# sea-with-sakura/ViT-of-Pytorch

Measured on AMD Instinct MI355X. Metric: images/sec training step, ViT-B/16 224px bf16, 1/2/4/8 MI355X, higher is better.
Workload: dtype bf16; 1 GPU; ViT-B16 @224 train step (fwd+CE+bwd+SGD-momentum/OneCycleLR); model=ViT-B16, image_size=224, per_gpu_batch=256, global_batch=256, seq_len=197, num_classes=1000, parallelism=dp1, step_launch=eager

## Files before the change

include/vit_hip.h:

```cpp
#ifndef VIT_HIP_H_
#define VIT_HIP_H_

#include <stdint.h>

#ifdef __cplusplus
extern "C" {
#endif

typedef void* vit_stream_t;

enum vit_status {
  VIT_OK = 0,
  VIT_ERR_INVALID_ARG = 1,
  VIT_ERR_HIP = 2,
  VIT_ERR_UNSUPPORTED = 3,
};

const char* vit_last_error(void);
int vit_abi_version(void);
const char* vit_build_id(void);

enum vit_layout { VIT_K_CONTIG = 0, VIT_MN_CONTIG = 1 };

typedef struct vit_dropout {
// ... 43 lines not shown
  int64_t batch;
  int64_t split_k;
  int64_t tokens;
  float* col_partial;
  int32_t epilogue;
  int32_t tile;
  const vit_dropout* dropout;
} vit_gemm_args;

int vit_gemm_bf16(const vit_gemm_args* args, vit_stream_t stream);
int64_t vit_gemm_tile_rows(const vit_gemm_args* args);
int64_t vit_gemm_partial_rows(const vit_gemm_args* args);
int64_t vit_gemm_split_rows(const vit_gemm_args* args);
int vit_gemm_bf16_part(const vit_gemm_args* args, int32_t part, vit_stream_t stream);
int vit_gemm_splitk_group(const vit_gemm_args* args, int32_t n, vit_stream_t stream);

int vit_splitk_reduce(const float* ws, int64_t batch, int64_t split, int64_t M, int64_t N,
                      float* out, int64_t ldo, int64_t out_batch_stride, int32_t accumulate,
                      vit_stream_t stream);
#define VIT_SPLITK_GROUP_MAX 8
typedef struct vit_splitk_job {
  const float* ws;
  int64_t batch, split, M, N;
  float* out;
  int64_t ldo, out_batch_stride;
  int32_t accumulate;
  int32_t reserved;
} vit_splitk_job;
int vit_splitk_reduce_group(const vit_splitk_job* jobs, int32_t njobs, vit_stream_t stream);

// ... 162 lines not shown
```

vit-of-pytorch_amd/csrc/capi.hip:

```cpp
#include <stdarg.h>

#include "common.h"
#include "build_id.h"

namespace vit {
static thread_local char g_last_error[512] = "";

void set_error(const char* fmt, ...) {
  va_list ap;
  va_start(ap, fmt);
  vsnprintf(g_last_error, sizeof(g_last_error), fmt, ap);
  va_end(ap);
}

int check_hip(hipError_t e, const char* what) {
  if (e == hipSuccess) return VIT_OK;
  set_error("%s: %s", what, hipGetErrorString(e));
  return VIT_ERR_HIP;
}
}

extern "C" const char* vit_last_error(void) { return vit::g_last_error; }
extern "C" int vit_abi_version(void) { return 20; }
extern "C" const char* vit_build_id(void) { return VIT_BUILD_ID; }
```

vit-of-pytorch_amd/csrc/gemm.hip:

```cpp
#include "gemm_decl.h"

namespace {
using vitg::GemmDev;
using vitg::EPI_DROP;

int pick_tile(const vit_gemm_args* a) {
  if (a->tile > 0) return (int)a->tile;
  const bool ak = a->a_layout == VIT_K_CONTIG, bk = a->b_layout == VIT_K_CONTIG;
  if (a->epilogue == VIT_EPI_SPLITK && a->M >= 256 && a->N >= 256) {
    static const int env_sk = vit::knob("VIT_GEMM_SPLITK_CFG", 9);
    return env_sk == 5 || env_sk == 6 || env_sk == 7 || env_sk == 8 ? env_sk : 9;
  }
  if (a->M >= 1024 && a->N >= 256) {
    static const int env_rs = vit::knob("VIT_GEMM_RESID_PP2", 1);
    if (ak && (env_rs || !(a->epilogue == VIT_EPI_BIAS_RESID_F32 && a->K < 2048))) return 9;
    if (a->N >= 2048 && a->epilogue != VIT_EPI_GELU_BWD && a->epilogue != VIT_EPI_MUL_BF16) return 5;
    if (!bk && a->K >= 3072) return 5;
    return 3;
  }
  return 0;
}

int tile_rows_of(int cfg) {
  switch (cfg) {
// ... 99 lines not shown
  d.B = (const char*)a->B; d.ldb = a->ldb; d.b_bs = a->b_batch_stride; d.b_bytes = (uint32_t)b_bytes;
  d.C = a->C; d.ldc = a->ldc; d.c_bs = a->c_batch_stride;
  d.C2 = a->C2; d.ldc2 = a->ldc2;
  d.bias = a->bias; d.bias_bs = a->bias_batch_stride;
  d.aux = a->aux; d.ldaux = a->ldaux; d.aux2 = a->aux2;
  d.split_k = (int)a->split_k; d.tokens = (int)a->tokens;
  {
    auto al = [](const void* q) { return ((uintptr_t)q % 32) == 0; };
    bool v = al(a->C) && a->ldc % 8 == 0 && a->c_batch_stride % 8 == 0;
    if (a->C2) v = v && al(a->C2) && a->ldc2 % 8 == 0;
    if (a->bias) v = v && al(a->bias) && a->bias_batch_stride % 8 == 0;
    if (a->aux) v = v && al(a->aux) && a->ldaux % 8 == 0;
    if (a->aux2) v = v && al(a->aux2);
    if (a->epilogue == VIT_EPI_SPLITK) v = al(a->C) && a->N % 8 == 0;
    d.vec = v ? 1 : 0;
  }
  d.col_partial = a->col_partial;
  d.drop = make_drop(a->dropout);
  VIT_CHECK_ARG(!d.drop.thr || a->epilogue == VIT_EPI_PATCH || a->epilogue == VIT_EPI_BIAS_RESID_F32 ||
                    a->epilogue == VIT_EPI_BIAS_GELU_DGELU,
                "vit_gemm_bf16: dropout is supported on the PATCH, BIAS_RESID_F32 and BIAS_GELU_DGELU epilogues");
  VIT_CHECK_ARG(!d.drop.thr || (a->a_layout == VIT_K_CONTIG &&
                                  (a->b_layout == VIT_K_CONTIG || a->epilogue == VIT_EPI_BIAS_RESID_F32)),
                "vit_gemm_bf16: dropout epilogues need a K-contiguous A (and B, except BIAS_RESID_F32)");
  {
    static const int env_gm = vit::knob("VIT_GEMM_GROUP_M", 8);
    static const int env_nt = vit::knob("VIT_GEMM_NT", 0);
    d.group_m = env_gm;
    d.nt = env_nt;
    static const int env_diag = vit::knob("VIT_GEMM_DIAG", 0);
// ... 98 lines not shown
    const vit_gemm_args* a = args + i;
    VIT_CHECK_ARG(a->epilogue == VIT_EPI_SPLITK && a->a_layout == VIT_MN_CONTIG && a->b_layout == VIT_MN_CONTIG &&
                      a->tile == 0 && !a->col_partial && !a->dropout,
                  "vit_gemm_splitk_group: member %d must be a split-K weight gradient (VIT_EPI_SPLITK, both operands "
                  "M/N-contiguous, no tile / col_partial / dropout)", i);
    bool empty = false;
    if (const int rc = make_dev(a, g.g[i], empty)) return rc;
    VIT_CHECK_ARG(!empty, "vit_gemm_splitk_group: member %d is empty", i);
    g.start[i] = (int)total;
    total += ((a->M + 255) / 256) * ((a->N + 255) / 256) * a->split_k * a->batch;
    VIT_CHECK_ARG(total < (1L << 30), "vit_gemm_splitk_group: grid too large");
  }
  g.start[n] = (int)total;
  g.n = n;
  return vit::check_hip(vitg::launch_splitk_group(g, (hipStream_t)stream), "vit_gemm_splitk_group launch");
}

namespace {
__global__ void splitk_reduce_kernel(const float* __restrict__ ws, int split, long M, long N, float* __restrict__ out,
                                     long ldo, long obs, int accumulate) {
  const int z = blockIdx.y;
  const long total = M * N;
  const float* w = ws + (long)z * split * total;
  float* o = out + z * obs;
  for (long i = (long)blockIdx.x * blockDim.x + threadIdx.x; i < total; i += (long)gridDim.x * blockDim.x) {
    float s = 0.f;
    for (int k = 0; k < split; ++k) s += w[k * total + i];
    const long m = i / N, n = i - m * N;
    float* dst = o + m * ldo + n;
    *dst = accumulate ? *dst + s : s;
// ... 135 lines not shown
```

vit-of-pytorch_amd/csrc/gemm_decl.h:

```cpp
#pragma once
#include "common.h"
#include <stdlib.h>

namespace vitg {

struct GemmDev {
  int M, N, K;
  const char* A;
  long lda;
  long a_bs;
  uint32_t a_bytes;
  const char* B;
  long ldb;
  long b_bs;
  uint32_t b_bytes;
  void* C;
  long ldc;
  long c_bs;
  void* C2;
  long ldc2;
  const float* bias;
  long bias_bs;
  const void* aux;
  long ldaux;
// ... 10 lines not shown
  int prio;
  int ilv;
#ifdef VIT_PP2_STAMPS
  unsigned long long* stamps;
#endif
};

constexpr int GEMM_GROUP_MAX = 4;
struct GemmGroup {
  GemmDev g[GEMM_GROUP_MAX];
  int start[GEMM_GROUP_MAX + 1];
  int n;
};
hipError_t launch_splitk_group(const GemmGroup& g, hipStream_t s);

constexpr int EPI_DROP = 16;

template <int EPI>
hipError_t launch_layout_x(int cfg, const GemmDev& d, bool ak, bool bk, int batch, int split, hipStream_t s);
template <int EPI>
hipError_t launch_kk_x(int cfg, const GemmDev& d, bool bk, int batch, int split, hipStream_t s);
template <> hipError_t launch_layout_x<0>(int, const GemmDev&, bool, bool, int, int, hipStream_t);
template <> hipError_t launch_layout_x<1>(int, const GemmDev&, bool, bool, int, int, hipStream_t);
template <> hipError_t launch_layout_x<2>(int, const GemmDev&, bool, bool, int, int, hipStream_t);
template <> hipError_t launch_layout_x<3>(int, const GemmDev&, bool, bool, int, int, hipStream_t);
template <> hipError_t launch_layout_x<4>(int, const GemmDev&, bool, bool, int, int, hipStream_t);
template <> hipError_t launch_layout_x<5>(int, const GemmDev&, bool, bool, int, int, hipStream_t);
template <> hipError_t launch_layout_x<6>(int, const GemmDev&, bool, bool, int, int, hipStream_t);
template <> hipError_t launch_layout_x<7>(int, const GemmDev&, bool, bool, int, int, hipStream_t);
template <> hipError_t launch_layout_x<8>(int, const GemmDev&, bool, bool, int, int, hipStream_t);
// ... 7 lines not shown
```

vit-of-pytorch_amd/csrc/gemm_e7.hip:

```cpp
#include "gemm_kernels.h"

template <> hipError_t vitg::launch_layout_x<7>(int cfg, const GemmDev& d, bool ak, bool bk, int batch, int split, hipStream_t s) {
  return launch_layout<7>(cfg, d, ak, bk, batch, split, s);
}

hipError_t vitg::launch_splitk_group(const GemmGroup& g, hipStream_t s) { return launch_pp2_group(g, s); }
```

vit-of-pytorch_amd/csrc/gemm_kernels.h:

```cpp
#pragma once
#include "gemm_decl.h"

namespace {
using vitg::GemmDev;
using vitg::GemmGroup;
using vitg::GEMM_GROUP_MAX;

__device__ __forceinline__ void tile_coords(int wg, int tiles_m, int tiles_n, int gm, int& tm, int& tn) {
  if (gm <= 1) {
    tm = wg / tiles_n;
    tn = wg % tiles_n;
    return;
  }
  const int per = gm * tiles_n;
  const int first = (wg / per) * gm;
  const int rows = tiles_m - first < gm ? tiles_m - first : gm;
  const int r = wg % per;
  tm = first + r % rows;
  tn = r / rows;
}

template <int BK>
__device__ __forceinline__ int swz_k(int row) {
  if constexpr (BK == 64) return (row >> 1) & 7;
// ... 148 lines not shown
    bf16_t* C = (bf16_t*)p.C + z * p.c_bs;
    const bf16_t* U = (const bf16_t*)p.aux;
    C[(long)m * p.ldc + n] = f2bf(v * bf2f(U[(long)m * p.ldaux + n]));
  } else if constexpr (E == VIT_EPI_PATCH) {
    float* C = (float*)p.C;
    const float* pos = (const float*)p.aux;
    const int t = m % p.tokens;
    float o;
    if (t == 0)
      o = p.aux2[n] + pos[n];
    else
      o = v + p.bias[n] + pos[(long)t * p.ldaux + n];
    if constexpr (DROP) o *= drop_mult1(p.drop, m, n);
    C[(long)m * p.ldc + n] = o;
  } else if constexpr (E == VIT_EPI_SPLITK) {
    float* C = (float*)p.C + ((long)z * p.split_k + split_idx) * (long)p.M * p.N;
    C[(long)m * p.N + n] = v;
  }
}

__device__ __forceinline__ void ld8f(const float* p, float* v) {
  const float4 a = *reinterpret_cast<const float4*>(p);
  const float4 b = *reinterpret_cast<const float4*>(p + 4);
  v[0] = a.x; v[1] = a.y; v[2] = a.z; v[3] = a.w; v[4] = b.x; v[5] = b.y; v[6] = b.z; v[7] = b.w;
}
typedef float v4f_t __attribute__((ext_vector_type(4)));
typedef unsigned v4u_t __attribute__((ext_vector_type(4)));
__device__ __forceinline__ void st8f(float* p, const float* v, bool nt = false) {
  const v4f_t a = {v[0], v[1], v[2], v[3]}, b = {v[4], v[5], v[6], v[7]};
  if (nt) {
    __builtin_nontemporal_store(a, reinterpret_cast<v4f_t*>(p));
    __builtin_nontemporal_store(b, reinterpret_cast<v4f_t*>(p + 4));
// ... 133 lines not shown
#pragma unroll
      for (int k = 0; k < 8; ++k) v[k] = b[k] + ps[k];
    } else {
      ld8f(p.bias + n, b);
#pragma unroll
      for (int k = 0; k < 8; ++k) v[k] += b[k] + ps[k];
    }
    if constexpr (DROP) {
      float dm[8];
      drop_mult8(p.drop, m, n >> 3, dm);
#pragma unroll
      for (int k = 0; k < 8; ++k) v[k] *= dm[k];
    }
    st8f((float*)p.C + (long)m * p.ldc + n, v, p.nt);
  } else if constexpr (E == VIT_EPI_SPLITK) {
    st8f((float*)p.C + ((long)z * p.split_k + split_idx) * (long)p.M * p.N + (long)m * p.N + n, v, p.nt);
  }
}

template <int EPI>
struct EpiOut {
  static constexpr int E = EPI & 15;
  static constexpr int W = (E == VIT_EPI_BF16 || E == VIT_EPI_BIAS_BF16 || E == VIT_EPI_GELU_BWD || E == VIT_EPI_MUL_BF16)
                               ? 1
                               : 2;
  static constexpr bool BIAS = E == VIT_EPI_BIAS_BF16 || E == VIT_EPI_BIAS_GELU || E == VIT_EPI_BIAS_RESID_F32 ||
                               E == VIT_EPI_BIAS_GELU_DGELU;
  static constexpr bool FAST = E != VIT_EPI_PATCH;
};

__device__ __forceinline__ uint4 pack8bf(const float* v) {
// ... 71 lines not shown
  }
}

__device__ __forceinline__ void st16(void* q, const uint4& x, bool nt) {
  const v4u_t u = {x.x, x.y, x.z, x.w};
  if (nt)
    __builtin_nontemporal_store(u, reinterpret_cast<v4u_t*>(q));
  else
    *reinterpret_cast<v4u_t*>(q) = u;
}

template <int EPI>
__device__ __forceinline__ void epi_put8(const GemmDev& p, int z, int split_idx, int m, int n, const uint4* o) {
  constexpr int E = EPI & 15;
  if constexpr (E == VIT_EPI_SPLITK) {
    float* q = (float*)p.C + ((long)z * p.split_k + split_idx) * (long)p.M * p.N + (long)m * p.N + n;
    st16(q, o[0], p.nt);
    st16(q + 4, o[1], p.nt);
  } else if constexpr (EpiOut<EPI>::W == 1) {
    st16((bf16_t*)p.C + z * p.c_bs + (long)m * p.ldc + n, o[0], p.nt);
  } else if constexpr (E == VIT_EPI_BIAS_GELU || E == VIT_EPI_BIAS_GELU_DGELU) {
    st16((bf16_t*)p.C + z * p.c_bs + (long)m * p.ldc + n, o[0], p.nt);
    st16((bf16_t*)p.C2 + z * p.c_bs + (long)m * p.ldc2 + n, o[1], p.nt);
  } else {
    float* q = (float*)p.C + z * p.c_bs + (long)m * p.ldc + n;
    st16(q, o[0], p.nt);
    st16(q + 4, o[1], p.nt);
  }
}

template <int EPI>
// ... 651 lines not shown
```

vit-of-pytorch_amd/csrc/gemm_pp2.inc:

```
template <bool AK, bool BKC, int EPI, int BK = 64, int NA = 2>
__device__ __forceinline__ void pp2_tile(const GemmDev& p, const int tm, const int tn, const int z,
                                         const int split_idx, const int orig) {
  constexpr int BM = 256, BN = 256, KK = BK / 32;
  constexpr int NB = NA + 1;
  constexpr int TN = BN / 4, FM = 8, FN = TN / 16;
  constexpr int HALF = 128 * BK * 2;
  constexpr int A0_OFF = 0, A1_OFF = NA * HALF, B_OFF = 2 * NA * HALF;
  constexpr int LDS = (2 * NA + 2 * NB) * HALF;
  constexpr int I = BK / 16;
  constexpr int LDW = TN + 4;
  constexpr int PR = 32;
  constexpr int WST = PR * LDW * 4;
  static_assert(8 * WST <= LDS && LDS <= 160 * 1024, "LDS budget / epilogue staging");
  static_assert(2 * I * (NA - 1) <= 32 && (2 * NA - 1) * I <= 62 && 2 * (NB - 1) * I <= 62, "vmcnt range");
  __shared__ __attribute__((aligned(16))) char smem[LDS];

  const int lane = threadIdx.x & 63;
  const int wave = __builtin_amdgcn_readfirstlane(threadIdx.x >> 6);
  const int grp = wave >> 2, wn = wave & 3;
  const int m0 = tm * BM, n0 = tn * BN;
  if (p.diag >= 100 && ((orig >> 3) & 1) && (orig >> 3) < 32) {
    const unsigned long long t0 = __builtin_amdgcn_s_memrealtime();
    while (__builtin_amdgcn_s_memrealtime() - t0 < (unsigned long long)(p.diag - 100) * 100ull)
      __builtin_amdgcn_s_sleep(8);
// ... 396 lines not shown
__global__ void __launch_bounds__(512) gemm_pp2_group_kernel(const GemmGroup G) {
  const int orig = blockIdx.x;
  const int w = xcd_major(orig, G.start[G.n]);
  int gi = 0;
#pragma unroll
  for (int k = 1; k < GEMM_GROUP_MAX; ++k)
    if (k < G.n && w >= G.start[k]) gi = k;
  gi = __builtin_amdgcn_readfirstlane(gi);
  const GemmDev& p = G.g[gi];
  const int tiles_m = (p.M + 255) / 256, tiles_n = (p.N + 255) / 256;
  int tm, tn, z, split_idx;
  splitk_coords(p, w - G.start[gi], tiles_m * tiles_n, tiles_m, tiles_n, tm, tn, z, split_idx);
  pp2_tile<AK, BKC, VIT_EPI_SPLITK>(p, tm, tn, z, split_idx, orig);
}

template <bool AK, bool BKC, int EPI, int BK = 64, int NA = 2>
hipError_t launch_pp2(const GemmDev& d, int batch, int split, hipStream_t s) {
  const int tiles = ((d.M + 255) / 256) * ((d.N + 255) / 256);
  dim3 grid(tiles, split, batch);
  hipLaunchKernelGGL((gemm_pp2_kernel<AK, BKC, EPI, BK, NA>), grid, dim3(512), 0, s, d);
  return hipGetLastError();
}

inline hipError_t launch_pp2_group(const GemmGroup& g, hipStream_t s) {
  hipLaunchKernelGGL((gemm_pp2_group_kernel<false, false>), dim3(g.start[g.n]), dim3(512), 0, s, g);
  return hipGetLastError();
}
```

vit-of-pytorch_amd/vitmi/_lib.py:

```python
from __future__ import annotations

import ctypes
import os

_HERE = os.path.dirname(os.path.abspath(__file__))
LIB_PATH = os.environ.get("VITMI_LIB") or os.path.join(_HERE, "libvit_hip.so")

c_i64 = ctypes.c_int64
c_i32 = ctypes.c_int32
c_f32 = ctypes.c_float
c_vp = ctypes.c_void_p

ABI_VERSION = 20

K_CONTIG, MN_CONTIG = 0, 1
(EPI_F32, EPI_BF16, EPI_BIAS_BF16, EPI_BIAS_GELU, EPI_BIAS_RESID_F32, EPI_GELU_BWD, EPI_PATCH, EPI_SPLITK,
 EPI_BIAS_GELU_DGELU, EPI_MUL_BF16) = range(10)


class Dropout(ctypes.Structure):
    _fields_ = [("p", c_f32), ("site", ctypes.c_uint32), ("seed", ctypes.c_uint64), ("offset", ctypes.c_uint64),
                ("row_stride", c_i64)]


class GemmArgs(ctypes.Structure):
    _fields_ = [
        ("M", c_i64), ("N", c_i64), ("K", c_i64),
        ("A", c_vp), ("lda", c_i64), ("a_batch_stride", c_i64),
# ... 28 lines not shown
    _fields_ = [("inp", c_vp), ("rows", c_i64), ("cols", c_i64), ("ldi", c_i64), ("out", c_vp), ("ldo", c_i64),
                ("rows_pad", c_i64), ("cols_pad", c_i64)]


CAST_BATCH_MAX = 8

_SIGS = {
    "vit_last_error": (ctypes.c_char_p, []),
    "vit_abi_version": (c_i32, []),
    "vit_gemm_bf16": (c_i32, [ctypes.POINTER(GemmArgs), c_vp]),
    "vit_gemm_tile_rows": (c_i64, [ctypes.POINTER(GemmArgs)]),
    "vit_gemm_partial_rows": (c_i64, [ctypes.POINTER(GemmArgs)]),
    "vit_gemm_split_rows": (c_i64, [ctypes.POINTER(GemmArgs)]),
    "vit_gemm_bf16_part": (c_i32, [ctypes.POINTER(GemmArgs), c_i32, c_vp]),
    "vit_gemm_splitk_group": (c_i32, [ctypes.POINTER(GemmArgs), c_i32, c_vp]),
    "vit_segment_colsum": (c_i32, [c_vp, c_i32, c_i64, c_i64, c_i64, c_i64, c_i64, c_i64, c_f32, c_vp, c_i64, c_vp]),
    "vit_segment_colsum_bcast": (c_i32, [c_vp, c_i32, c_i64, c_i64, c_i64, c_i64, c_i64, c_i64, c_f32, c_vp, c_i64,
                                         c_vp, c_i64, c_i64, c_vp]),
    "vit_router_dx_gate_partial_rows": (c_i64, [c_i64]),
    "vit_router_dx_gate": (c_i32, [c_vp, c_i64, c_vp, c_i64, c_f32, c_vp, c_i64, c_i64, c_i64, c_i64, c_i64, c_vp,
                                   c_i64, c_i64, c_i64, c_vp, c_i64, c_vp]),
    "vit_splitk_reduce_group": (c_i32, [ctypes.POINTER(SplitkJob), c_i32, c_vp]),
    "vit_cast_pad_batch": (c_i32, [ctypes.POINTER(CastJob), c_i32, c_vp]),
    "vit_router_head_partials": (c_i64, [c_i64]),
    "vit_cast_rows_masked": (c_i32, [c_vp, c_i64, c_i64, c_i64, c_vp, c_vp, c_i64, c_vp]),
    "vit_router_select": (c_i32, [c_vp, c_i64, c_i32, ctypes.POINTER(ctypes.c_uint32), c_i32, c_vp, c_vp, c_vp, c_vp]),
    "vit_cls_mse": (c_i32, [c_vp, c_i64, c_vp, c_i64, c_i64, c_i64, c_vp, c_vp, c_vp, c_vp]),
    "vit_cls_mse_bwd": (c_i32, [c_vp, c_i64, c_vp, c_i64, c_i64, c_vp, c_vp]),
    "vit_router_head_fwd": (c_i32, [c_vp, c_vp, c_i32, c_vp, c_i64, c_i64, c_i32, c_i64, c_i32, c_f32, c_vp, c_vp, c_vp,
                                    c_vp, c_vp, c_vp, c_vp]),
# ... 111 lines not shown
```

vit-of-pytorch_amd/vitmi/engine.py:

```python
from __future__ import annotations

import math
import os
from collections import OrderedDict
from dataclasses import dataclass

import torch

from . import ops
from ._lib import (EPI_BF16, EPI_BIAS_BF16, EPI_BIAS_GELU_DGELU, EPI_BIAS_RESID_F32, EPI_MUL_BF16, EPI_PATCH,
                   EPI_SPLITK, K_CONTIG, MN_CONTIG)

ALIGN = 64


def _rup(x, m):
    return (x + m - 1) // m * m


_NBUF = 2

_WGRAD_TARGET = int(os.environ.get("VIT_WGRAD_TARGET", "256"))


# ... 148 lines not shown
        self.dqkv = [z(Tp, 3 * D), z(Tp, 3 * D)]
        self.dlncls = z(b, D, dt=f)
        self.dlogits = z(b, cfg.num_classes, dt=f)
        self.row_stats = z(b, 3, dt=f)
        self.lnparts = [z(ops.layernorm_bwd_blocks(T), 3 * D, dt=f) for _ in range(_NBUF)]
        self.gelu_parts = [z(-(-T // 128), M, dt=f) for _ in range(_NBUF)]
        self.attn_bias_rows = ops.attention_bias_rows(N, D // H)
        self.qkv_bparts = [z(b * self.attn_bias_rows, 3 * D, dt=f) for _ in range(_NBUF)]
        nws = ops.attention_workspace_elems(b, N, H)
        self.attn_ws = z(nws, dt=f) if nws else None
        bp = _rup(b, 64)
        self.bp = bp
        self.c_o, self.c_ln2, self.c_dh, self.c_dh2, self.c_dyln = (z(bp, D) for _ in range(5))
        self.c_g, self.c_gp, self.c_dg = (z(bp, M) for _ in range(3))
        self.c_mu2, self.c_rs2 = z(b, dt=f), z(b, dt=f)


class _BiasReducer:

    def __init__(self, eng, a):
        self.eng = eng
        self.a = a
        self.D = eng.cfg.emb_dim
        self.nxt = {}
        self.queued = {}
        self.jobs = []

    def buf(self, kind, bufs):
        n = self.queued.get(kind, 0)
        if n == len(bufs):
# ... 47 lines not shown
        self.wqkv = torch.zeros(L, D, 3 * D, device=self.dev, dtype=bf)
        self.bqkv = torch.zeros(L, 3 * D, device=self.dev)
        kp = _rup(cfg.patch_k, 64)
        self.wconv = torch.zeros(D, kp, device=self.dev, dtype=torch.bfloat16) if kp != cfg.patch_k else None
        self._acts = {}
        self._mirror_sig = None
        o = [self.off(self.lname(i, "norm1.weight")) for i in range(L)]
        self.layer_stride = o[0] - o[1] if L > 1 else 0
        assert all(o[i] == o[0] - i * self.layer_stride for i in range(L))
        self._ws = None
        self.step_id = 0
        self.grad_ready_hook = None
        self.grad_ready_finish = None
        self.overlap_wgrad = os.environ.get("VITMI_OVERLAP", "0") == "1"
        self.group_wgrad = os.environ.get("VITMI_GROUP_WGRAD", "1") != "0"
        self.prune_last = os.environ.get("VITMI_PRUNE_LAST", "1") != "0"
        self._pruned = False
        self._side = None
        self._ev_pool, self._ev_next = [], 0
        self.probe = None
        self.probe_wgrad = None
        self.drop_seed = (torch.initial_seed() * 0x9E3779B97F4A7C15 + 0x632BE59BD9B4E019) & (2**64 - 1)
        self._drop_offset = 0
        self._drop = None

    def _event(self):
        if self._ev_next == len(self._ev_pool):
            self._ev_pool.append(torch.cuda.Event())
        ev = self._ev_pool[self._ev_next]
        self._ev_next += 1
# ... 79 lines not shown
            A, lda, B, ldb, M, N, _, _, _, batch, b_bs, _ = sp
            w = ws[o:o + n]
            o += n
            views.append(w)
            members.append((A, B, w, M, N, K, dict(a_layout=MN_CONTIG, b_layout=MN_CONTIG, lda=lda, ldb=ldb, ldc=N,
                                                    epilogue=EPI_SPLITK, batch=batch, b_bs=b_bs, split_k=s)))
        if self.probe_wgrad is not None:
            ev0 = torch.cuda.Event(enable_timing=True)
            ev0.record()
        ops.gemm_splitk_group(members)
        if self.probe_wgrad is not None:
            ev1 = torch.cuda.Event(enable_timing=True)
            ev1.record()
            self.probe_wgrad.append((ev0, ev1, sum(2.0 * sp[4] * sp[5] * K * sp[9] for sp in specs), K, True))
        ops.splitk_reduce_group([(w, sp[9], s, sp[4], sp[5], sp[7], sp[8], sp[11], False) for sp, w in zip(specs, views)])

    def _dd(self, site, row_stride=1):
        if self._drop is None:
            return None
        p, seed, off = self._drop
        return ops.dropout_desc(p, site, seed, off, row_stride)

    def forward(self, x: torch.Tensor, dropout_p: float = 0.0):
        cfg = self.cfg
        if x.dim() != 4 or x.shape[1] != 3 or tuple(x.shape[2:]) != cfg.image_hw:
            raise ValueError(f"expected input [b, 3, {cfg.image_hw[0]}, {cfg.image_hw[1]}], got {tuple(x.shape)}")
        x = x.to(self.dev, torch.float32).contiguous()
        b = x.shape[0]
        a = self.acts(b)
        D, M, H, N, L = cfg.emb_dim, cfg.mlp_dim, cfg.num_heads, cfg.tokens, cfg.num_layers
# ... 185 lines not shown
                main.wait_event(ev)

        def fire(bucket):
            bias.flush()
            if not hook:
                return
            evs = []
            for st in ((main, side) if overlap else (main,)):
                ev = self._event()
                ev.record(st)
                evs.append(ev)
            hook(g, *bucket, evs)

        self._ev_next = 0
        group = self.group_wgrad and D >= 256
        out_wb = None
        bias = _BiasReducer(self, a)
        ops.gemm_f32(C, D, b, dl, C, True, a.lncls, D, False, gv("classifier.weight"), D)
        bias.reduce(dl, b, C, C, (gv("classifier.bias"),))
        ops.gemm_f32(b, D, C, dl, C, False, f[self.off("classifier.weight"):], D, False, a.dlncls, D)
        wb = 0
        pruned = self._pruned
        ops.zero_(a.dh)
        if not pruned:
            ops.zero_(a.dhb[wb])
        bias.ln_bwd(a.dlncls, D, a.h[L], N * D, a.muf, a.rsf, f[self.off("transformer.norm.weight"):], a.dh, N * D, b,
                    gv("transformer.norm.weight"), gv(self.lname(L - 1, "mlp.fc2.bias")),
                    dx_bf16=a.c_dh if pruned else a.dhb[wb], lddxb=D if pruned else N * D,
                    dx_dropout=dd(3 + 3 * (L - 1), N))
        fire(self.layout.buckets[0])
        scale = 1.0 / math.sqrt(hd)
        for i in reversed(range(L)):
            ln = lambda s: self.off(self.lname(i, s))
            li = i & 1
            if pruned and i == L - 1:
                self._backward_last_cls(a, i, b, g, on_side, bias)
                wb ^= 1
            else:
                dhb = a.dhb[wb]
                on_side(lambda: self._wgrad(dhb, D, a.g[i], M, D, M, a.Tp, gv(self.lname(i, "mlp.fc2.weight")), M))
                release("dhb", wb)
                dg = a.dg[li]
                acquire("dg", li)
                gpart = bias.buf("gelu", a.gelu_parts)
                w2 = mv[ln("mlp.fc2.weight"):]
                kw = dict(a_layout=K_CONTIG, b_layout=MN_CONTIG, lda=D, ldb=M, ldc=M, epilogue=EPI_MUL_BF16, aux=a.gp[i],
                          ldaux=M, col_partial=gpart)
                ops.gemm(dhb, w2, dg, T, M, D, **kw)
                tiles_m = ops.gemm_partial_rows(dhb, w2, dg, T, M, D, **kw)
                bias.reduce(gpart, tiles_m, M, M, (gv(self.lname(i, "mlp.fc1.bias")),))
                on_side(lambda: self._wgrad(dg, M, a.ln2[i], D, M, D, a.Tp, gv(self.lname(i, "mlp.fc1.weight")), D))
                release("dg", li)
                ops.gemm(dg, mv[ln("mlp.fc1.weight"):], a.dyln, T, D, M, a_layout=K_CONTIG, b_layout=MN_CONTIG, lda=M,
                         ldb=D, ldc=D, epilogue=EPI_BF16)
                wb ^= 1
                acquire("dhb", wb)
                dhb = a.dhb[wb]
                bias.ln_bwd(a.dyln, D, a.hm[i], D, a.mu2[i], a.rs2[i], f[ln("norm2.weight"):], a.dh, D, T,
                            gv(self.lname(i, "norm2.weight")), gv(self.lname(i, "attn.out.bias")),
                            dres=a.dh, lddres=D, dx_bf16=dhb, lddxb=D, dx_dropout=dd(1 + 3 * i))
                out_spec = (a.o[i], D, dhb, D, D, D, a.Tp, gv(self.lname(i, "attn.out.weight")), D, 1, 0, 0)
                if group:
                    out_wb = wb
                else:
                    on_side(lambda: self._wgrad(*out_spec[:9]))
                    release("dhb", wb)
                ops.gemm(dhb, mv[ln("attn.out.weight"):], a.dO, T, D, D, a_layout=K_CONTIG, b_layout=K_CONTIG, lda=D,
                         ldb=D, ldc=D, epilogue=EPI_BF16)
            dqkv = a.dqkv[li]
            acquire("dqkv", li)
            qpart = bias.buf("qkv", a.qkv_bparts)
            ops.attention_bwd(a.qkv[i], a.o[i], a.dO, a.lse[i], dqkv, b, N, H, hd, scale, bias_partial=qpart,
                              q_rows=1 if pruned and i == L - 1 else None, workspace=a.attn_ws)
            qo = ln("attn.query.weight")
            zs = ln("attn.key.weight") - qo
            qb = ln("attn.query.bias")
            bias.reduce(qpart, b * a.attn_bias_rows, 3 * D, 3 * D, (g[qb:], g[qb + zs:], g[qb + 2 * zs:]), seg=D)
            qkv_spec = (a.ln1[i], D, dqkv, 3 * D, D, D, a.Tp, g[qo:], D, 3, D, zs)
            if out_wb is not None:
                on_side(lambda: self._wgrad_group([out_spec, qkv_spec]))
                release("dqkv", li)
                release("dhb", out_wb)
                out_wb = None
            else:
                on_side(lambda: self._wgrad(*qkv_spec[:9], batch=3, b_bs=D, out_bs=zs))
                release("dqkv", li)
            ops.gemm(dqkv, self.wqkv[i], a.dyln, T, D, 3 * D, a_layout=K_CONTIG, b_layout=K_CONTIG, lda=3 * D,
                     ldb=3 * D, ldc=D, epilogue=EPI_BF16)
            wb ^= 1
            acquire("dhb", wb)
            bias.ln_bwd(a.dyln, D, a.h[i], D, a.mu1[i], a.rs1[i], f[ln("norm1.weight"):], a.dh, D, T,
                        gv(self.lname(i, "norm1.weight")), gv(self.lname(i - 1, "mlp.fc2.bias")) if i > 0 else None,
                        dres=a.dh, lddres=D, dx_bf16=a.dhb[wb], lddxb=D,
                        dx_dropout=dd(3 + 3 * (i - 1)) if i > 0 else dd(0))
            fire(self.layout.buckets[L - i])
        dhb = a.dhb[wb]
        on_side(lambda: self._wgrad(dhb, D, a.patches, a.kpad, D, cfg.patch_k, a.Tp, gv("embedding.weight"),
                                    cfg.patch_k))
        ops.embed_grad(a.dh, b, N, D, gv("transformer.pos_embedding.pos_embedding"), gv("cls_token"),
                       gv("embedding.bias"), dropout=dd(0))
        fire(self.layout.buckets[-1])
        bias.flush()
        if overlap:
            main.wait_stream(side)
        return g
```

vit-of-pytorch_amd/vitmi/ops.py:

```python
from __future__ import annotations

import ctypes

import torch

from . import _lib
from ._lib import COLSUM_BATCH_MAX, Dropout, GemmArgs, check

BF16 = torch.bfloat16
F32 = torch.float32


def lib():
    return _lib.load()


def _stream():
    return ctypes.c_void_p(torch.cuda.current_stream().cuda_stream)


def _p(t):
    return ctypes.c_void_p(0 if t is None else t.data_ptr())


# ... 502 lines not shown
            best, best_t = s, t
    return best


def gemm_splitk_group(members):
    if not 1 <= len(members) <= 4:
        raise ValueError("gemm_splitk_group: 1 to 4 members")
    arr = (GemmArgs * len(members))()
    for i, (A, B, C, M, N, K, kw) in enumerate(members):
        _chk(A, BF16, "A")
        _chk(B, BF16, "B")
        arr[i] = _gemm_args(A, B, C, M, N, K, **kw)
    check(lib().vit_gemm_splitk_group(arr, len(members), _stream()), "vit_gemm_splitk_group")


def splitk_factor(M, N, K, batch=1, cus=256):
    tile = 256 if M >= 256 and N >= 256 else 128
    slots = cus if tile == 256 else 2 * cus
    tiles = -(-M // tile) * -(-N // tile) * batch
    smax = max(1, min((K // 64) // 8, 32))
    t_tile = 2.0 * tile * tile * K / 4.0e12
    slab = 2.0 * M * N * 4 * batch / 5.0e12
    best, best_t = 1, None
    for s in range(1, smax + 1):
        t = -(-tiles * s // slots) * t_tile / s + s * slab
        if best_t is None or t < best_t * (1 - 1e-9):
            best, best_t = s, t
    return best


# ... 28 lines not shown
```

Baseline: 7711 images/sec.

## Defer all weight-gradient GEMMs into one table-driven grouped launch

Weight-gradient GEMMs are no longer launched per layer during backward. They are queued and issued at the end as one grouped kernel. The kernel reads a device-resident table of per-member GEMM descriptors, which is cached across steps and keyed on pointers, and each workgroup finds its member by binary search. Split-K members can now write directly into the gradient buffer through ldc and c_bs. The aim is to cut launch overhead and fill the device with one large grid, at the cost of extra per-layer activation-gradient buffers, serialising wgrad after the dgrad chain, and a host sync whenever the table is rebuilt.

Measured after the change: 7824 images/sec, median of 6. 1.01x the previous value.

```diff
diff --git a/include/vit_hip.h b/include/vit_hip.h
--- a/include/vit_hip.h
+++ b/include/vit_hip.h
@@ -81,6 +81,11 @@
 int64_t vit_gemm_split_rows(const vit_gemm_args* args);
 int vit_gemm_bf16_part(const vit_gemm_args* args, int32_t part, vit_stream_t stream);
 int vit_gemm_splitk_group(const vit_gemm_args* args, int32_t n, vit_stream_t stream);
+#define VIT_GEMM_TABLE_MAX 128
+int64_t vit_gemm_group_table_bytes(int32_t n);
+int vit_gemm_group_prepare(const vit_gemm_args* args, const int32_t* direct, int32_t n, void* table,
+                           int64_t table_bytes, int32_t* total, vit_stream_t stream);
+int vit_gemm_group_launch(const void* table, int32_t n, int32_t total, vit_stream_t stream);
 
 int vit_splitk_reduce(const float* ws, int64_t batch, int64_t split, int64_t M, int64_t N,
                       float* out, int64_t ldo, int64_t out_batch_stride, int32_t accumulate,
diff --git a/vit-of-pytorch_amd/csrc/capi.hip b/vit-of-pytorch_amd/csrc/capi.hip
--- a/vit-of-pytorch_amd/csrc/capi.hip
+++ b/vit-of-pytorch_amd/csrc/capi.hip
@@ -21,5 +21,5 @@
 }
 
 extern "C" const char* vit_last_error(void) { return vit::g_last_error; }
-extern "C" int vit_abi_version(void) { return 20; }
+extern "C" int vit_abi_version(void) { return 21; }
 extern "C" const char* vit_build_id(void) { return VIT_BUILD_ID; }
diff --git a/vit-of-pytorch_amd/csrc/gemm.hip b/vit-of-pytorch_amd/csrc/gemm.hip
--- a/vit-of-pytorch_amd/csrc/gemm.hip
+++ b/vit-of-pytorch_amd/csrc/gemm.hip
@@ -1,4 +1,6 @@
 #include "gemm_decl.h"
+
+#include <vector>
 
 namespace {
 using vitg::GemmDev;
@@ -137,6 +139,10 @@
     if (a->aux2) v = v && al(a->aux2);
     if (a->epilogue == VIT_EPI_SPLITK) v = al(a->C) && a->N % 8 == 0;
     d.vec = v ? 1 : 0;
+  }
+  if (a->epilogue == VIT_EPI_SPLITK) {
+    d.ldc = a->N;
+    d.c_bs = a->M * a->N;
   }
   d.col_partial = a->col_partial;
   d.drop = make_drop(a->dropout);
@@ -265,6 +271,58 @@
   g.start[n] = (int)total;
   g.n = n;
   return vit::check_hip(vitg::launch_splitk_group(g, (hipStream_t)stream), "vit_gemm_splitk_group launch");
+}
+
+extern "C" int64_t vit_gemm_group_table_bytes(int32_t n) {
+  return n >= 1 && n <= vitg::GEMM_TABLE_MAX ? (int64_t)vitg::group_table_bytes(n) : 0;
+}
+
+extern "C" int vit_gemm_group_prepare(const vit_gemm_args* args, const int32_t* direct, int32_t n, void* table,
+                                      int64_t table_bytes, int32_t* total_out, vit_stream_t stream) {
+  VIT_CHECK_ARG(args != nullptr && n >= 1 && n <= vitg::GEMM_TABLE_MAX, "vit_gemm_group_prepare: 1..%d members, got %d",
+                vitg::GEMM_TABLE_MAX, n);
+  VIT_CHECK_ARG(table != nullptr && total_out != nullptr && table_bytes >= (int64_t)vitg::group_table_bytes(n) &&
+                    ((uintptr_t)table % 16) == 0,
+                "vit_gemm_group_prepare: needs a 16-byte aligned table of vit_gemm_group_table_bytes(n) bytes");
+  const size_t soff = vitg::group_table_start_off(n);
+  std::vector<char> host(vitg::group_table_bytes(n), 0);
+  GemmDev* g = reinterpret_cast<GemmDev*>(host.data());
+  int* start = reinterpret_cast<int*>(host.data() + soff);
+  long total = 0;
+  for (int i = 0; i < n; ++i) {
+    const vit_gemm_args* a = args + i;
+    VIT_CHECK_ARG(a->epilogue == VIT_EPI_SPLITK && a->a_layout == VIT_MN_CONTIG && a->b_layout == VIT_MN_CONTIG &&
+                      a->tile == 0 && !a->col_partial && !a->dropout,
+                  "vit_gemm_group_prepare: member %d must be a split-K weight gradient (VIT_EPI_SPLITK, both operands "
+                  "M/N-contiguous, no tile / col_partial / dropout)", i);
+    bool empty = false;
+    if (const int rc = make_dev(a, g[i], empty)) return rc;
+    VIT_CHECK_ARG(!empty, "vit_gemm_group_prepare: member %d is empty", i);
+    if (direct && direct[i]) {
+      VIT_CHECK_ARG(a->split_k == 1 && a->ldc >= a->N && (a->batch == 1 || a->c_batch_stride > 0),
+                    "vit_gemm_group_prepare: direct member %d needs split_k 1, ldc >= N and an output batch stride", i);
+      g[i].ldc = a->ldc;
+      g[i].c_bs = a->c_batch_stride;
+      g[i].vec = ((uintptr_t)a->C % 32) == 0 && a->ldc % 8 == 0 && a->c_batch_stride % 8 == 0;
+    }
+    start[i] = (int)total;
+    total += ((a->M + 255) / 256) * ((a->N + 255) / 256) * a->split_k * a->batch;
+    VIT_CHECK_ARG(total < (1L << 30), "vit_gemm_group_prepare: grid too large");
+  }
+  start[n] = (int)total;
+  hipStream_t s = (hipStream_t)stream;
+  if (const int rc = vit::check_hip(hipStreamSynchronize(s), "vit_gemm_group_prepare sync")) return rc;
+  if (const int rc = vit::check_hip(hipMemcpy(table, host.data(), host.size(), hipMemcpyHostToDevice),
+                                    "vit_gemm_group_prepare upload"))
+    return rc;
+  *total_out = (int32_t)total;
+  return VIT_OK;
+}
+
+extern "C" int vit_gemm_group_launch(const void* table, int32_t n, int32_t total, vit_stream_t stream) {
+  VIT_CHECK_ARG(table != nullptr && n >= 1 && n <= vitg::GEMM_TABLE_MAX && total >= 1,
+                "vit_gemm_group_launch: a prepared table, its member count and its workgroup total");
+  return vit::check_hip(vitg::launch_group_table(table, n, total, (hipStream_t)stream), "vit_gemm_group_launch");
 }
 
 namespace {
diff --git a/vit-of-pytorch_amd/csrc/gemm_decl.h b/vit-of-pytorch_amd/csrc/gemm_decl.h
--- a/vit-of-pytorch_amd/csrc/gemm_decl.h
+++ b/vit-of-pytorch_amd/csrc/gemm_decl.h
@@ -48,6 +48,11 @@
 };
 hipError_t launch_splitk_group(const GemmGroup& g, hipStream_t s);
 
+constexpr int GEMM_TABLE_MAX = 128;
+inline size_t group_table_start_off(int n) { return ((size_t)n * sizeof(GemmDev) + 15) & ~(size_t)15; }
+inline size_t group_table_bytes(int n) { return group_table_start_off(n) + ((size_t)n + 1) * sizeof(int); }
+hipError_t launch_group_table(const void* table, int n, int total, hipStream_t s);
+
 constexpr int EPI_DROP = 16;
 
 template <int EPI>
diff --git a/vit-of-pytorch_amd/csrc/gemm_e7.hip b/vit-of-pytorch_amd/csrc/gemm_e7.hip
--- a/vit-of-pytorch_amd/csrc/gemm_e7.hip
+++ b/vit-of-pytorch_amd/csrc/gemm_e7.hip
@@ -5,3 +5,7 @@
 }
 
 hipError_t vitg::launch_splitk_group(const GemmGroup& g, hipStream_t s) { return launch_pp2_group(g, s); }
+
+hipError_t vitg::launch_group_table(const void* table, int n, int total, hipStream_t s) {
+  return launch_pp2_table(table, n, total, s);
+}
diff --git a/vit-of-pytorch_amd/csrc/gemm_kernels.h b/vit-of-pytorch_amd/csrc/gemm_kernels.h
--- a/vit-of-pytorch_amd/csrc/gemm_kernels.h
+++ b/vit-of-pytorch_amd/csrc/gemm_kernels.h
@@ -186,8 +186,8 @@
     if constexpr (DROP) o *= drop_mult1(p.drop, m, n);
     C[(long)m * p.ldc + n] = o;
   } else if constexpr (E == VIT_EPI_SPLITK) {
-    float* C = (float*)p.C + ((long)z * p.split_k + split_idx) * (long)p.M * p.N;
-    C[(long)m * p.N + n] = v;
+    float* C = (float*)p.C + ((long)z * p.split_k + split_idx) * p.c_bs;
+    C[(long)m * p.ldc + n] = v;
   }
 }
 
@@ -351,7 +351,7 @@
     }
     st8f((float*)p.C + (long)m * p.ldc + n, v, p.nt);
   } else if constexpr (E == VIT_EPI_SPLITK) {
-    st8f((float*)p.C + ((long)z * p.split_k + split_idx) * (long)p.M * p.N + (long)m * p.N + n, v, p.nt);
+    st8f((float*)p.C + ((long)z * p.split_k + split_idx) * p.c_bs + (long)m * p.ldc + n, v, p.nt);
   }
 }
 
@@ -453,7 +453,7 @@
 __device__ __forceinline__ void epi_put8(const GemmDev& p, int z, int split_idx, int m, int n, const uint4* o) {
   constexpr int E = EPI & 15;
   if constexpr (E == VIT_EPI_SPLITK) {
-    float* q = (float*)p.C + ((long)z * p.split_k + split_idx) * (long)p.M * p.N + (long)m * p.N + n;
+    float* q = (float*)p.C + ((long)z * p.split_k + split_idx) * p.c_bs + (long)m * p.ldc + n;
     st16(q, o[0], p.nt);
     st16(q + 4, o[1], p.nt);
   } else if constexpr (EpiOut<EPI>::W == 1) {
diff --git a/vit-of-pytorch_amd/csrc/gemm_pp2.inc b/vit-of-pytorch_amd/csrc/gemm_pp2.inc
--- a/vit-of-pytorch_amd/csrc/gemm_pp2.inc
+++ b/vit-of-pytorch_amd/csrc/gemm_pp2.inc
@@ -434,6 +434,27 @@
   pp2_tile<AK, BKC, VIT_EPI_SPLITK>(p, tm, tn, z, split_idx, orig);
 }
 
+template <bool AK, bool BKC>
+__global__ void __launch_bounds__(512) gemm_pp2_table_kernel(const GemmDev* __restrict__ tab,
+                                                             const int* __restrict__ start, const int n) {
+  const int orig = blockIdx.x;
+  const int w = xcd_major(orig, (int)gridDim.x);
+  int lo = 0, hi = n;
+  while (hi - lo > 1) {
+    const int mid = (lo + hi) >> 1;
+    if (w >= start[mid])
+      lo = mid;
+    else
+      hi = mid;
+  }
+  const int gi = __builtin_amdgcn_readfirstlane(lo);
+  const GemmDev p = tab[gi];
+  const int tiles_m = (p.M + 255) / 256, tiles_n = (p.N + 255) / 256;
+  int tm, tn, z, split_idx;
+  splitk_coords(p, w - start[gi], tiles_m * tiles_n, tiles_m, tiles_n, tm, tn, z, split_idx);
+  pp2_tile<AK, BKC, VIT_EPI_SPLITK>(p, tm, tn, z, split_idx, orig);
+}
+
 template <bool AK, bool BKC, int EPI, int BK = 64, int NA = 2>
 hipError_t launch_pp2(const GemmDev& d, int batch, int split, hipStream_t s) {
   const int tiles = ((d.M + 255) / 256) * ((d.N + 255) / 256);
@@ -446,3 +467,10 @@
   hipLaunchKernelGGL((gemm_pp2_group_kernel<false, false>), dim3(g.start[g.n]), dim3(512), 0, s, g);
   return hipGetLastError();
 }
+
+inline hipError_t launch_pp2_table(const void* table, int n, int total, hipStream_t s) {
+  const GemmDev* tab = (const GemmDev*)table;
+  const int* start = (const int*)((const char*)table + vitg::group_table_start_off(n));
+  hipLaunchKernelGGL((gemm_pp2_table_kernel<false, false>), dim3(total), dim3(512), 0, s, tab, start, n);
+  return hipGetLastError();
+}
diff --git a/vit-of-pytorch_amd/vitmi/_lib.py b/vit-of-pytorch_amd/vitmi/_lib.py
--- a/vit-of-pytorch_amd/vitmi/_lib.py
+++ b/vit-of-pytorch_amd/vitmi/_lib.py
@@ -11,7 +11,7 @@
 c_f32 = ctypes.c_float
 c_vp = ctypes.c_void_p
 
-ABI_VERSION = 20
+ABI_VERSION = 21
 
 K_CONTIG, MN_CONTIG = 0, 1
 (EPI_F32, EPI_BF16, EPI_BIAS_BF16, EPI_BIAS_GELU, EPI_BIAS_RESID_F32, EPI_GELU_BWD, EPI_PATCH, EPI_SPLITK,
@@ -70,6 +70,10 @@
     "vit_gemm_split_rows": (c_i64, [ctypes.POINTER(GemmArgs)]),
     "vit_gemm_bf16_part": (c_i32, [ctypes.POINTER(GemmArgs), c_i32, c_vp]),
     "vit_gemm_splitk_group": (c_i32, [ctypes.POINTER(GemmArgs), c_i32, c_vp]),
+    "vit_gemm_group_table_bytes": (c_i64, [c_i32]),
+    "vit_gemm_group_prepare": (c_i32, [ctypes.POINTER(GemmArgs), ctypes.POINTER(c_i32), c_i32, c_vp, c_i64,
+                                       ctypes.POINTER(c_i32), c_vp]),
+    "vit_gemm_group_launch": (c_i32, [c_vp, c_i32, c_i32, c_vp]),
     "vit_segment_colsum": (c_i32, [c_vp, c_i32, c_i64, c_i64, c_i64, c_i64, c_i64, c_i64, c_f32, c_vp, c_i64, c_vp]),
     "vit_segment_colsum_bcast": (c_i32, [c_vp, c_i32, c_i64, c_i64, c_i64, c_i64, c_i64, c_i64, c_f32, c_vp, c_i64,
                                          c_vp, c_i64, c_i64, c_vp]),
diff --git a/vit-of-pytorch_amd/vitmi/engine.py b/vit-of-pytorch_amd/vitmi/engine.py
--- a/vit-of-pytorch_amd/vitmi/engine.py
+++ b/vit-of-pytorch_amd/vitmi/engine.py
@@ -186,6 +186,18 @@
         self.c_o, self.c_ln2, self.c_dh, self.c_dh2, self.c_dyln = (z(bp, D) for _ in range(5))
         self.c_g, self.c_gp, self.c_dg = (z(bp, M) for _ in range(3))
         self.c_mu2, self.c_rs2 = z(b, dt=f), z(b, dt=f)
+        self._cfg, self._dev = cfg, dev
+        self.dhb_l = self.dg_l = self.dqkv_l = None
+
+    def defer_bufs(self):
+        if self.dhb_l is None:
+            cfg = self._cfg
+            D, M, L = cfg.emb_dim, cfg.mlp_dim, cfg.num_layers
+            z = lambda *s: torch.zeros(*s, device=self._dev, dtype=torch.bfloat16)
+            self.dhb_l = self.dhb + [z(self.Tp, D) for _ in range(2 * L - 1)]
+            self.dg_l = self.dg + [z(self.Tp, M) for _ in range(max(L - 2, 0))]
+            self.dqkv_l = self.dqkv + [z(self.Tp, 3 * D) for _ in range(max(L - 2, 0))]
+        return self.dhb_l, self.dg_l, self.dqkv_l
 
 
 class _BiasReducer:
@@ -263,6 +275,9 @@
         self.grad_ready_finish = None
         self.overlap_wgrad = os.environ.get("VITMI_OVERLAP", "0") == "1"
         self.group_wgrad = os.environ.get("VITMI_GROUP_WGRAD", "1") != "0"
+        v = os.environ.get("VITMI_WGRAD_DEFER", "all")
+        self.wgrad_defer = L if v == "all" else int(v)
+        self._wgrad_tables = {}
         self.prune_last = os.environ.get("VITMI_PRUNE_LAST", "1") != "0"
         self._pruned = False
         self._side = None
@@ -372,6 +387,47 @@
             ev1.record()
             self.probe_wgrad.append((ev0, ev1, sum(2.0 * sp[4] * sp[5] * K * sp[9] for sp in specs), K, True))
         ops.splitk_reduce_group([(w, sp[9], s, sp[4], sp[5], sp[7], sp[8], sp[11], False) for sp, w in zip(specs, views)])
+
+    def _wgrad_batch(self, specs, slot):
+        K = specs[0][6]
+        assert all(sp[6] == K for sp in specs)
+        s = ops.splitk_factor_group([(sp[4], sp[5], sp[9]) for sp in specs], K, _WGRAD_TARGET)
+        views = None
+        if s > 1:
+            sizes = [sp[9] * s * sp[4] * sp[5] for sp in specs]
+            ws = self._workspace(sum(sizes))
+            views, o = [], 0
+            for n in sizes:
+                views.append(ws[o:o + n])
+                o += n
+        for c0 in range(0, len(specs), ops.GEMM_TABLE_MAX):
+            part = specs[c0:c0 + ops.GEMM_TABLE_MAX]
+            key = (s, self._ws.data_ptr() if s > 1 else 0) + tuple(
+                (sp[0].data_ptr(), sp[1], sp[2].data_ptr(), sp[3], sp[4], sp[5], sp[7].data_ptr()) + tuple(sp[8:])
+                for sp in part)
+            ent = self._wgrad_tables.get((self._last_b, slot, c0))
+            if ent is None or ent[0] != key:
+                members = []
+                for k, (A, lda, B, ldb, M, N, _, out, ldo, batch, b_bs, out_bs) in enumerate(part):
+                    kw = dict(a_layout=MN_CONTIG, b_layout=MN_CONTIG, lda=lda, ldb=ldb, epilogue=EPI_SPLITK, batch=batch,
+                              b_bs=b_bs, split_k=s)
+                    if s == 1:
+                        members.append((A, B, out, M, N, K, dict(kw, ldc=ldo, c_bs=out_bs), True))
+                    else:
+                        members.append((A, B, views[c0 + k], M, N, K, dict(kw, ldc=N), False))
+                ent = (key, ops.GemmGroupTable(members))
+                self._wgrad_tables[(self._last_b, slot, c0)] = ent
+            if self.probe_wgrad is not None:
+                ev0 = torch.cuda.Event(enable_timing=True)
+                ev0.record()
+            ent[1].launch()
+            if self.probe_wgrad is not None:
+                ev1 = torch.cuda.Event(enable_timing=True)
+                ev1.record()
+                self.probe_wgrad.append((ev0, ev1, sum(2.0 * sp[4] * sp[5] * K * sp[9] for sp in part), K, True))
+        if s > 1:
+            ops.splitk_reduce_group([(w, sp[9], s, sp[4], sp[5], sp[7], sp[8], sp[11], False)
+                                     for sp, w in zip(specs, views)])
 
     def _dd(self, site, row_stride=1):
         if self._drop is None:
@@ -587,6 +643,17 @@
 
         self._ev_next = 0
         group = self.group_wgrad and D >= 256
+        defer = self.wgrad_defer if not hook and not overlap and D >= 256 and M >= 256 else 0
+        pending, held, launches = [], 0, 0
+        dhbs, dgs, dqkvs = a.defer_bufs() if defer else (a.dhb, a.dg, a.dqkv)
+        nd = len(dhbs)
+
+        def flush_wgrad():
+            nonlocal pending, held, launches
+            if pending:
+                self._wgrad_batch(pending, launches)
+                launches += 1
+            pending, held = [], 0
         out_wb = None
         bias = _BiasReducer(self, a)
         ops.gemm_f32(C, D, b, dl, C, True, a.lncls, D, False, gv("classifier.weight"), D)
@@ -596,24 +663,27 @@
         pruned = self._pruned
         ops.zero_(a.dh)
         if not pruned:
-            ops.zero_(a.dhb[wb])
+            ops.zero_(dhbs[wb])
         bias.ln_bwd(a.dlncls, D, a.h[L], N * D, a.muf, a.rsf, f[self.off("transformer.norm.weight"):], a.dh, N * D, b,
                     gv("transformer.norm.weight"), gv(self.lname(L - 1, "mlp.fc2.bias")),
-                    dx_bf16=a.c_dh if pruned else a.dhb[wb], lddxb=D if pruned else N * D,
+                    dx_bf16=a.c_dh if pruned else dhbs[wb], lddxb=D if pruned else N * D,
                     dx_dropout=dd(3 + 3 * (L - 1), N))
         fire(self.layout.buckets[0])
         scale = 1.0 / math.sqrt(hd)
         for i in reversed(range(L)):
             ln = lambda s: self.off(self.lname(i, s))
-            li = i & 1
+            li = i % len(dgs)
             if pruned and i == L - 1:
                 self._backward_last_cls(a, i, b, g, on_side, bias)
-                wb ^= 1
+                wb = (wb + 1) % nd
             else:
-                dhb = a.dhb[wb]
-                on_side(lambda: self._wgrad(dhb, D, a.g[i], M, D, M, a.Tp, gv(self.lname(i, "mlp.fc2.weight")), M))
+                dhb = dhbs[wb]
+                if defer:
+                    pending.append((dhb, D, a.g[i], M, D, M, a.Tp, gv(self.lname(i, "mlp.fc2.weight")), M, 1, 0, 0))
+                else:
+                    on_side(lambda: self._wgrad(dhb, D, a.g[i], M, D, M, a.Tp, gv(self.lname(i, "mlp.fc2.weight")), M))
                 release("dhb", wb)
-                dg = a.dg[li]
+                dg = dgs[li]
                 acquire("dg", li)
                 gpart = bias.buf("gelu", a.gelu_parts)
                 w2 = mv[ln("mlp.fc2.weight"):]
@@ -622,25 +692,30 @@
                 ops.gemm(dhb, w2, dg, T, M, D, **kw)
                 tiles_m = ops.gemm_partial_rows(dhb, w2, dg, T, M, D, **kw)
                 bias.reduce(gpart, tiles_m, M, M, (gv(self.lname(i, "mlp.fc1.bias")),))
-                on_side(lambda: self._wgrad(dg, M, a.ln2[i], D, M, D, a.Tp, gv(self.lname(i, "mlp.fc1.weight")), D))
+                if defer:
+                    pending.append((dg, M, a.ln2[i], D, M, D, a.Tp, gv(self.lname(i, "mlp.fc1.weight")), D, 1, 0, 0))
+                else:
+                    on_side(lambda: self._wgrad(dg, M, a.ln2[i], D, M, D, a.Tp, gv(self.lname(i, "mlp.fc1.weight")), D))
                 release("dg", li)
                 ops.gemm(dg, mv[ln("mlp.fc1.weight"):], a.dyln, T, D, M, a_layout=K_CONTIG, b_layout=MN_CONTIG, lda=M,
                          ldb=D, ldc=D, epilogue=EPI_BF16)
-                wb ^= 1
+                wb = (wb + 1) % nd
                 acquire("dhb", wb)
-                dhb = a.dhb[wb]
+                dhb = dhbs[wb]
                 bias.ln_bwd(a.dyln, D, a.hm[i], D, a.mu2[i], a.rs2[i], f[ln("norm2.weight"):], a.dh, D, T,
                             gv(self.lname(i, "norm2.weight")), gv(self.lname(i, "attn.out.bias")),
                             dres=a.dh, lddres=D, dx_bf16=dhb, lddxb=D, dx_dropout=dd(1 + 3 * i))
                 out_spec = (a.o[i], D, dhb, D, D, D, a.Tp, gv(self.lname(i, "attn.out.weight")), D, 1, 0, 0)
-                if group:
+                if defer:
+                    pending.append(out_spec)
+                elif group:
                     out_wb = wb
                 else:
                     on_side(lambda: self._wgrad(*out_spec[:9]))
                     release("dhb", wb)
                 ops.gemm(dhb, mv[ln("attn.out.weight"):], a.dO, T, D, D, a_layout=K_CONTIG, b_layout=K_CONTIG, lda=D,
                          ldb=D, ldc=D, epilogue=EPI_BF16)
-            dqkv = a.dqkv[li]
+            dqkv = dqkvs[li]
             acquire("dqkv", li)
             qpart = bias.buf("qkv", a.qkv_bparts)
             ops.attention_bwd(a.qkv[i], a.o[i], a.dO, a.lse[i], dqkv, b, N, H, hd, scale, bias_partial=qpart,
@@ -650,7 +725,12 @@
             qb = ln("attn.query.bias")
             bias.reduce(qpart, b * a.attn_bias_rows, 3 * D, 3 * D, (g[qb:], g[qb + zs:], g[qb + 2 * zs:]), seg=D)
             qkv_spec = (a.ln1[i], D, dqkv, 3 * D, D, D, a.Tp, g[qo:], D, 3, D, zs)
-            if out_wb is not None:
+            if defer:
+                pending.append(qkv_spec)
+                held += 1
+                if held == defer and i > 0:
+                    flush_wgrad()
+            elif out_wb is not None:
                 on_side(lambda: self._wgrad_group([out_spec, qkv_spec]))
                 release("dqkv", li)
                 release("dhb", out_wb)
@@ -660,16 +740,20 @@
                 release("dqkv", li)
             ops.gemm(dqkv, self.wqkv[i], a.dyln, T, D, 3 * D, a_layout=K_CONTIG, b_layout=K_CONTIG, lda=3 * D,
                      ldb=3 * D, ldc=D, epilogue=EPI_BF16)
-            wb ^= 1
+            wb = (wb + 1) % nd
             acquire("dhb", wb)
             bias.ln_bwd(a.dyln, D, a.h[i], D, a.mu1[i], a.rs1[i], f[ln("norm1.weight"):], a.dh, D, T,
                         gv(self.lname(i, "norm1.weight")), gv(self.lname(i - 1, "mlp.fc2.bias")) if i > 0 else None,
-                        dres=a.dh, lddres=D, dx_bf16=a.dhb[wb], lddxb=D,
+                        dres=a.dh, lddres=D, dx_bf16=dhbs[wb], lddxb=D,
                         dx_dropout=dd(3 + 3 * (i - 1)) if i > 0 else dd(0))
             fire(self.layout.buckets[L - i])
-        dhb = a.dhb[wb]
-        on_side(lambda: self._wgrad(dhb, D, a.patches, a.kpad, D, cfg.patch_k, a.Tp, gv("embedding.weight"),
-                                    cfg.patch_k))
+        dhb = dhbs[wb]
+        if defer and cfg.patch_k >= 256:
+            pending.append((dhb, D, a.patches, a.kpad, D, cfg.patch_k, a.Tp, gv("embedding.weight"), cfg.patch_k, 1, 0, 0))
+        else:
+            on_side(lambda: self._wgrad(dhb, D, a.patches, a.kpad, D, cfg.patch_k, a.Tp, gv("embedding.weight"),
+                                        cfg.patch_k))
+        flush_wgrad()
         ops.embed_grad(a.dh, b, N, D, gv("transformer.pos_embedding.pos_embedding"), gv("cls_token"),
                        gv("embedding.bias"), dropout=dd(0))
         fire(self.layout.buckets[-1])
diff --git a/vit-of-pytorch_amd/vitmi/ops.py b/vit-of-pytorch_amd/vitmi/ops.py
--- a/vit-of-pytorch_amd/vitmi/ops.py
+++ b/vit-of-pytorch_amd/vitmi/ops.py
@@ -540,6 +540,34 @@
     check(lib().vit_gemm_splitk_group(arr, len(members), _stream()), "vit_gemm_splitk_group")
 
 
+GEMM_TABLE_MAX = 128
+
+
+class GemmGroupTable:
+
+    def __init__(self, members):
+        n = len(members)
+        if not 1 <= n <= GEMM_TABLE_MAX:
+            raise ValueError(f"GemmGroupTable: 1 to {GEMM_TABLE_MAX} members")
+        arr = (GemmArgs * n)()
+        direct = (ctypes.c_int32 * n)()
+        for i, (A, B, C, M, N, K, kw, d) in enumerate(members):
+            _chk(A, BF16, "A")
+            _chk(B, BF16, "B")
+            _chk(C, F32, "C")
+            arr[i] = _gemm_args(A, B, C, M, N, K, **kw)
+            direct[i] = int(bool(d))
+        nbytes = int(lib().vit_gemm_group_table_bytes(n))
+        self.table = torch.empty(nbytes, device=members[0][0].device, dtype=torch.uint8)
+        total = ctypes.c_int32(0)
+        check(lib().vit_gemm_group_prepare(arr, direct, n, _p(self.table), nbytes, ctypes.byref(total), _stream()),
+              "vit_gemm_group_prepare")
+        self.n, self.total = n, int(total.value)
+
+    def launch(self):
+        check(lib().vit_gemm_group_launch(_p(self.table), self.n, self.total, _stream()), "vit_gemm_group_launch")
+
+
 def splitk_factor(M, N, K, batch=1, cus=256):
     tile = 256 if M >= 256 and N >= 256 else 128
     slots = cus if tile == 256 else 2 * cus
```
